# mhnazeri/PMoE

Hardware: AMD Instinct MI355X
Metric: samples/sec fwd+bwd, 256x256 RGB 4-expert PMoE (higher is better)
Workload: dtype bf16; 1 GPU; 4-expert MoE (PMoE experts), 256x256x3 x4 frames, batch 64/GPU, fwd+moe_loss+bwd, dropout 0.3; global_batch=64, parallelism=dp1

## Files before the change

include/pmoe_hip.h:

```cpp
#ifndef PMOE_HIP_H
#define PMOE_HIP_H
#include <stdint.h>
#ifdef __cplusplus
extern "C" {
#endif

#define PMOE_DT_BF16 0
#define PMOE_DT_F32 1

#define PMOE_ERR_ARG (-1)
#define PMOE_ERR_UNSUPPORTED (-2)

#define PMOE_ACT_NONE 0
#define PMOE_ACT_RELU 1
#define PMOE_ACT_ELU 2
#define PMOE_ACT_TANH 3
#define PMOE_ACT_SIGMOID 4

#define PMOE_RES_NONE 0
#define PMOE_RES_ADD 1
#define PMOE_RES_DRELU 2
#define PMOE_RES_DELU 3
#define PMOE_RES_DTANH 4
#define PMOE_RES_DSIGMOID 5
// ... 90 lines not shown
                  float* part, int32_t nparts, float* shiftc, int32_t dtype, void* stream);
int pmoe_reduce_partials(const float* part_in, float* part_out, int32_t E, int32_t nin, int32_t nout, int32_t width,
                         void* stream);
int pmoe_bn_finalize(const float* part, int32_t nparts, int64_t count, const void* const* gamma_ptrs,
                     const void* const* beta_ptrs, void* const* rmean_ptrs, void* const* rvar_ptrs, float momentum,
                     float eps, int32_t training, float* scale, float* shift, float* mean, float* invstd, int32_t E,
                     int32_t C, const float* shiftc, void* stream);
int pmoe_bn_apply(const void* x, const void* res, void* y, const float* scale, const float* shift, const float* mean,
                  int64_t rows_per_expert, int32_t E, int32_t C, int32_t relu, int32_t y_ld, int32_t y_coff,
                  int32_t dtype, void* y_fp8, float in_scale, void* stream);
int pmoe_bn_apply_gap(const void* x, void* y, const float* scale, const float* shift, const float* mean, float* gap_part,
                      int32_t nparts, int32_t N, int32_t ipe, int64_t HW, int32_t C, int32_t relu, int32_t dtype, void* stream);
int pmoe_bn_bwd_reduce(const void* dy, const void* y, const void* x, const float* mean, const float* invstd,
                       const float* scale, const float* shift, int64_t rows_per_expert, int32_t E, int32_t C, int32_t relu, float* part, int32_t nparts,
                       void* gmask_out, int32_t dtype, void* stream);
int pmoe_bn_bwd_finalize(const float* part, int32_t nparts, int64_t count, float* dgamma, float* dbeta, float* c1,
                         float* c2, int32_t E, int32_t C, void* stream);
int pmoe_bn_apply_pool2(const void* x, void* y, void* pooled, const float* scale, const float* shift, const float* mean,
                        int32_t ipe, int32_t H, int32_t W, int32_t E, int32_t C, int32_t relu, int32_t y_ld, int32_t y_coff,
                        int32_t dtype, void* stream);
int pmoe_bn_bwd_apply(const void* dy, const void* y, const void* x, const float* mean, const float* invstd,
                      const float* scale, const float* shift, const float* c1, const float* c2, void* dx, void* gmask_out,
                      int64_t rows_per_expert, int32_t E, int32_t C, int32_t relu, int32_t dtype, void* stream);

int pmoe_maxpool3s2_fwd(const void* x, void* y, uint8_t* argmax, int32_t N, int32_t H, int32_t W, int32_t C,
                        int32_t dtype, void* stream);
int pmoe_maxpool3s2_bwd(const void* dy, const uint8_t* argmax, void* dx, int32_t N, int32_t H, int32_t W, int32_t C,
                        int32_t dtype, void* stream);
int pmoe_gap_partial(const void* a, const void* b, float* part, int32_t N, int64_t HW, int32_t C, int32_t nparts,
                     int32_t b_shared_ipe, int32_t dtype, void* stream);
int pmoe_gap_finish(const float* part, void* out, int32_t N, int32_t C, int32_t nparts, int64_t HW, int32_t out_ld,
                    int32_t out_coff, int32_t dtype, void* stream);
int pmoe_gap_bwd(const void* g, void* dx, int32_t N, int64_t HW, int32_t C, int32_t g_ld, int32_t g_coff,
                 int32_t dtype, void* stream);

int pmoe_stem_tail_stats(const void* z2, const float* sc2, const float* sh2, const float* mu2, float* part,
                         int32_t nparts, float* shiftc, float* part_x, int32_t E, int32_t ipe, int32_t H, int32_t W,
                         int32_t C, int32_t dtype, void* stream);
int pmoe_stem_tail_pool(const void* z2, void* y, uint8_t* argmax, const float* sc2, const float* sh2, const float* sc1,
                        const float* sh1, const float* mu2, const float* mu1, int32_t N, int32_t ipe, int32_t H, int32_t W, int32_t C, int32_t dtype,
                        void* stream);
int pmoe_stem_tail_bwd(int32_t phase, const void* z2, const void* dpool, const uint8_t* argmax, void* dz2,
                       const float* const* consts, float* part, int32_t nparts, int32_t E, int32_t ipe, int32_t H,
                       int32_t W, int32_t C, int32_t dtype, void* stream);
int pmoe_stem_tail_pooled(const void* y, const void* dpool, const uint8_t* argmax, const float* const* consts,
                          float* part4, int32_t nparts, int32_t E, int64_t rows_per_expert, int32_t C, int32_t dtype,
// ... 107 lines not shown
```

pmoe_amd/csrc/elementwise.hip:

```cpp
#include "common.h"

#define DISPATCH_DT(dtype, CALL)                      \
    do {                                              \
        if ((dtype) == PMOE_DT_BF16) { using T = bf16; CALL; } \
        else if ((dtype) == PMOE_DT_F32) { using T = float; CALL; } \
        else return PMOE_ERR_ARG;                     \
    } while (0)

static inline bool pow2(int v) { return v > 0 && !(v & (v - 1)); }

template <typename T, int MODE>
__global__ void __launch_bounds__(256) colstats_kernel(const T* __restrict__ x, const T* __restrict__ dy,
                                                      const T* __restrict__ y, const float* __restrict__ mean,
                                                      const float* __restrict__ invstd, const float* __restrict__ scale,
                                                      const float* __restrict__ shift, long long rpe, int C, int ld,
                                                      int coff, int relu, float* __restrict__ part, int nparts,
                                                      float* __restrict__ shiftc, T* __restrict__ gmask) {
    constexpr int VE = 16 / (int)sizeof(T);
    const int CV = C / VE, RL = 256 / CV;
    const int tid = threadIdx.x, cv = tid % CV, rl = tid / CV;
    const int e = blockIdx.y, pi = blockIdx.x;
    const long long rpp = (rpe + nparts - 1) / nparts;
    long long r0 = (long long)pi * rpp, r1 = r0 + rpp;
    if (r1 > rpe) r1 = rpe;
// ... 249 lines not shown
    }
    const bool remask = relu && !y;
    for (long long i = i0; i < nvec; i += (long long)gridDim.x * 256) {
        const size_t off = ebase + (size_t)i * VE;
        float gv[VE], xv[VE], o[VE];
        unpack16<T>(ldg16(dy + off), gv);
        unpack16<T>(ldg16(x + off), xv);
        if (remask) {
#pragma unroll
            for (int k = 0; k < VE; ++k) gv[k] = ((xv[k] - mu[k]) * sc[k] + sh[k]) > 0.f ? gv[k] : 0.f;
        } else if (relu) {
            float yv[VE];
            unpack16<T>(ldg16(y + off), yv);
#pragma unroll
            for (int k = 0; k < VE; ++k) gv[k] = yv[k] > 0.f ? gv[k] : 0.f;
        }
#pragma unroll
        for (int k = 0; k < VE; ++k) o[k] = gv[k] * A[k] + ((xv[k] - mu[k]) * Bx[k] + K[k]);
        stg16(dx + off, pack16<T>(o));
        if (gm) stg16(gm + off, pack16<T>(gv));
    }
}

template <typename T>
__global__ void __launch_bounds__(256) bn_apply_pool2_kernel(const T* __restrict__ x, T* __restrict__ y, T* __restrict__ pooled,
                                                            const float* __restrict__ scale, const float* __restrict__ shift,
                                                            const float* __restrict__ mean, int ipe, int H, int W, int C, int relu,
                                                            int y_ld, int y_coff) {
    constexpr int VE = 16 / (int)sizeof(T);
    const int CV = C / VE;
    const int e = blockIdx.y, Ho = H / 2, Wo = W / 2;
    const long long nq = (long long)ipe * Ho * Wo * CV;
    const long long i0 = (long long)blockIdx.x * 256 + threadIdx.x;
    const int cv = (int)(i0 % CV);
    float sc[VE], sh[VE], mu[VE];
#pragma unroll
    for (int k = 0; k < VE; ++k) {
        sc[k] = scale[e * C + cv * VE + k]; sh[k] = shift[e * C + cv * VE + k]; mu[k] = mean[e * C + cv * VE + k];
    }
    const size_t rpe = (size_t)ipe * H * W;
    for (long long i = i0; i < nq; i += (long long)gridDim.x * 256) {
        long long t = i / CV;
        const int ox = (int)(t % Wo); t /= Wo;
        const int oy = (int)(t % Ho);
        const int n = (int)(t / Ho);
        const size_t r00 = (size_t)e * rpe + ((size_t)n * H + 2 * oy) * W + 2 * ox;
// ... 485 lines not shown
        const long long nq = (long long)ipe * (H / 2) * (W / 2) * (C / VE);
        hipLaunchKernelGGL((bn_apply_pool2_kernel<T>), dim3(grid_for(nq, 2048), E), dim3(256), 0, (hipStream_t)stream, (const T*)x,
                           (T*)y, (T*)pooled, scale, shift, mean, ipe, H, W, C, relu, y_ld, y_coff);
        return (int)hipGetLastError();
    });
}

int pmoe_bn_bwd_apply(const void* dy, const void* y, const void* x, const float* mean, const float* invstd,
                      const float* scale, const float* shift, const float* c1, const float* c2, void* dx, void* gmask_out,
                      int64_t rows_per_expert, int32_t E, int32_t C, int32_t relu, int32_t dtype, void* stream) {
    DISPATCH_DT(dtype, {
        constexpr int VE = 16 / (int)sizeof(T);
        if (C % VE || !pow2(C / VE) || C / VE > 256) return PMOE_ERR_ARG;
        const long long nvec = rows_per_expert * (C / VE);
        int cap = 1024 / (E > 0 ? E : 1);
        cap = cap < 64 ? 64 : cap;
        hipLaunchKernelGGL((bn_bwd_apply_kernel<T>), dim3(grid_for(nvec, cap), E), dim3(256), 0, (hipStream_t)stream,
                           (const T*)dy, (const T*)y, (const T*)x, mean, invstd, scale, shift, c1, c2, (T*)dx, (T*)gmask_out,
                           (long long)rows_per_expert, C, relu);
        return (int)hipGetLastError();
    });
}

int pmoe_act_fwd(const void* x, void* y, int64_t n, int32_t act, float drop_p, uint64_t seed, int32_t dtype, void* stream) {
    if (!x || !y || n <= 0 || act < PMOE_ACT_NONE || act > PMOE_ACT_SIGMOID || drop_p < 0.f || drop_p >= 1.f) return PMOE_ERR_ARG;
    DISPATCH_DT(dtype, {
        constexpr int VE = 16 / (int)sizeof(T);
        if (n % VE) return PMOE_ERR_ARG;
        hipLaunchKernelGGL((act_fwd_kernel<T>), dim3(grid_for(n / VE)), dim3(256), 0, (hipStream_t)stream, (const T*)x, (T*)y,
                           (long long)(n / VE), act, drop_p, (unsigned long long)seed);
        return (int)hipGetLastError();
    });
}

int pmoe_act_bwd(const void* dy, const void* y, void* dx, int64_t n, int32_t act, float drop_p, int32_t dtype, void* stream) {
    if (!dy || !y || !dx || n <= 0 || act < PMOE_ACT_NONE || act > PMOE_ACT_SIGMOID || drop_p < 0.f || drop_p >= 1.f) return PMOE_ERR_ARG;
    DISPATCH_DT(dtype, {
        constexpr int VE = 16 / (int)sizeof(T);
        if (n % VE) return PMOE_ERR_ARG;
        hipLaunchKernelGGL((act_bwd_kernel<T>), dim3(grid_for(n / VE)), dim3(256), 0, (hipStream_t)stream, (const T*)dy,
                           (const T*)y, (T*)dx, (long long)(n / VE), act, drop_p);
        return (int)hipGetLastError();
    });
}

int pmoe_maxpool3s2_fwd(const void* x, void* y, uint8_t* argmax, int32_t N, int32_t H, int32_t W, int32_t C,
// ... 136 lines not shown
```

pmoe_amd/engine.py:

```python
import itertools
import os

import torch
import torch.distributed as dist

from . import hip, ops
from .model import blocks as B
from .parallel import BucketedAllReduce

F32 = torch.float32


def r16(c):
    return (c + 15) // 16 * 16


def r64(c):
    return (c + 63) // 64 * 64


class Var:
    __slots__ = ("t", "coff", "c", "g", "needs_grad", "act", "drop_p", "base", "gap_part", "bn_src", "bn_part", "f8", "bn_defer",
                 "bn_fused", "pending_bn")

# ... 105 lines not shown
    def __init__(self, experts, alt=False, shared_k=0):
        self.experts = list(experts)
        self.E = len(self.experts)
        self.alt = alt
        self.shared = shared_k > 0
        self.K = shared_k if self.shared else self.E
        if self.shared and (self.E != 1 or alt or 5 * self.K > 64):
            raise ValueError("shared-trunk mixture: one trunk, plain alpha head, n_experts <= 12")
        self.dp_group = None
        self.dp_enabled = False
        self.dp_buckets = 6
        self.dp_always = False
        self._built_for = None
        self._seed_counter = itertools.count(1)
        self.fuse_conv_stats = True
        self.fuse_stem_tail = True
        self.fold_stem_input = True
        self.overlap_wgrad = os.environ.get("PMOE_OVERLAP_WGRAD", "0") == "1"
        self.fold_bn_eval = True
        self.pooled_stem_bwd = True
        self.fold_eca_gate = True
        self.bn_mask_in_reduce = os.environ.get("PMOE_BN_MASK_IN_REDUCE", "1") != "0"
        self.bn_reduce_in_dgrad = os.environ.get("PMOE_BN_REDUCE_IN_DGRAD", "1") != "0"
        self.fuse_bn_gap = os.environ.get("PMOE_FUSE_BN_GAP", "1") != "0"
        self.stem_bn_fuse = os.environ.get("PMOE_STEM_BN_FUSE", "1") != "0"
        self.mlp_wgrad_fused = os.environ.get("PMOE_MLP_WGRAD", "1") != "0"
        self.fp8 = False
        self.fp8_in_scale = 16.0
        self.fp8_min_cin = int(os.environ.get("PMOE_FP8_MIN_CIN", "64"))
        self.raw_alpha = False
        self.debug_grads = None
        self.debug_acts = None
        self._collect()

    def _collect(self):
        ex = self.experts
        self.params = []

        def conv(name, mods, ks=None):
            m0 = mods[0]
            if isinstance(m0, B.Linear):
                layer = GroupedConv(self, name, [m.weight for m in mods],
                                    [m.bias for m in mods] if m0.bias is not None else None,
                                    m0.in_features, m0.out_features, 1, 1, 0)
            else:
                layer = GroupedConv(self, name, [m.weight for m in mods],
# ... 472 lines not shown
        if gm is not None:
            if dz is not None:
                ops.set_meta(name=layer.name, bytes=nb * 3)
                ops.bn_bwd_apply(gm, None, z.t, mean, invstd, scale, shift, c1, c2, dz, None, rpe, E, C_, False)
        else:
            gm = torch.empty_like(z.t) if want_res else None
            if dz is None and gm is None:
                return
            if dz is None:
                dz = torch.empty_like(z.t)
            ops.set_meta(name=layer.name, bytes=nb * (2 + (ysrc is not None) + 1 + (gm is not None)))
            ops.bn_bwd_apply(dy, ysrc, z.t, mean, invstd, scale, shift, c1, c2, dz, gm, rpe, E, C_, relu)
        if self.debug_grads is not None:
            self.debug_grads[layer.name + ":dz"] = dz.detach().clone()
            self.debug_grads[layer.name + ":stats"] = (mean.clone(), invstd.clone(), c1.clone(), c2.clone())
        if z.needs_grad:
            if z.grad is not None:
                raise RuntimeError("BN input consumed twice")
            z.set_grad(dz)
        if want_res:
            if res.grad is not None:
                raise RuntimeError("residual gradient slot already filled")
            res.set_grad(gm)

    def _bn_grad_views(self, layer):
        return (self._grad_slot("gamma", layer).view(self.E, layer.C), self._grad_slot("beta", layer).view(self.E, layer.C),
                None)

    def _stem_tail(self, z2, stats):
        E, C_ = self.E, self.bn_c2.C
        n, h, w, _ = z2.t.shape
        rpe = self.B * h * w
        sc2, sh2, mu2, is2 = self._bn_coeffs(self.bn_c2, rpe, stats, stats.shape[0] // E if stats is not None else 0, z2)
        nparts = self._nparts(rpe)
        part = part_x = None
        if self.training:
            part = torch.empty(E, nparts, 2, C_, dtype=F32, device=self.dev)
            shc = torch.empty(E, C_, dtype=F32, device=self.dev)
            if self.taping:
                part_x = torch.empty(E, nparts, 3, C_, dtype=F32, device=self.dev)
            ops.stem_tail_stats(z2.t, sc2, sh2, mu2, part, nparts, E, self.B, shiftc=shc, part_x=part_x)
            if part_x is not None:
                part_x, npx = self._fold_parts(part_x, nparts, 3 * C_)
        sc1, sh1, mu1, is1 = self._bn_coeffs(self.bn1, rpe, part, nparts, shiftc=shc if self.training else None)
        ho, wo = (h - 1) // 2 + 1, (w - 1) // 2 + 1
        y = Var(self._new(n, ho, wo, C_))
# ... 320 lines not shown
            z1.needs_grad = True
            z1.bn_defer = (self.stem_bn_fuse and self.training and self.bn_reduce_in_dgrad and self.dtype == torch.bfloat16
                           and fold2 and ops.conv2d_wgrad(x0.t, z1.t, None, cin=self.conv1.cinp, cout=self.conv1.cout_st,
                                                          cinp=64, coutp=64, ipe=self.B, ks=3, stride=1, pad=self.conv1.pad,
                                                          x_shared=True, per_image=True, bn_fuse=(z1.t, None, None, None),
                                                          plan_only=True) == 7209)
            self.tape.append(lambda: self._stem_in_bwd(x0, z1, gate, gapmean))
            a1 = self._bn(z1, self.bn_c1, relu=True, stats=st, want_gap=fold2)
        else:
            x0s = self._eca(x0, self.eca1, shared=True)
            a1 = self._conv_bn(x0s, self.conv1, self.bn_c1, relu=True)
        if fold2:
            z2, st = self._eca_conv_folded(a1, self.eca2, self.conv2)
        else:
            a1s = self._eca(a1, self.eca2, shared=False)
            z2, st = self._conv_stats(a1s, self.conv2)
        if self.fuse_stem_tail:
            o = self._stem_tail(z2, st)
        else:
            a2 = self._bn(z2, self.bn_c2, relu=True, stats=st)
            a3 = self._bn(a2, self.bn1, relu=True)
            o = self._maxpool(a3)
        for bi, blk in enumerate(self.blocks):
            idn = o
            if blk["down"] is not None:
                idn = self._conv_bn(o, blk["down"][0], blk["down"][1], relu=False)
            nxt = self.blocks[bi + 1]["conv1"] if bi + 1 < len(self.blocks) else None
            aA = self._conv_bn(o, blk["conv1"], blk["bn1"], relu=True, want_f8=blk["conv2"].fp8)
            o = self._conv_bn(aA, blk["conv2"], blk["bn2"], relu=True, res=idn, want_f8=nxt is not None and nxt.fp8)
        self._gap_to(o, feat, 0)

    def _conv_bn(self, x, conv, bn, relu, res=None, out=None, want_f8=False, pool_to=None):
        if self.training or self.taping or not self.fold_bn_eval or conv.w_f8 is not None:
            z, st = self._conv_stats(x, conv)
            return self._bn(z, bn, relu=relu, res=res, stats=st, out=out, want_f8=want_f8, pool_to=pool_to)
        E = self.E
        key = (self.dtype, str(self.dev)) + tuple(p._version for p in conv.weights) + tuple(
            v for m in bn.mods for v in (m.weight._version, m.bias._version, m.running_mean._version, m.running_var._version))
        cache = conv.__dict__.get("_bn_fold")
        if cache is None or cache[0] != key:
            scale, shift, mean, _ = self._bn_coeffs(bn, 1)
            wf = torch.empty(E, conv.coutp, conv.taps, conv.cinp, dtype=self.dtype, device=self.dev)
            bf = torch.empty(E, conv.coutp, dtype=F32, device=self.dev)
            ops.pack_conv_weights_scaled(self._tab("w", conv), scale, shift, mean, wf, bf, E, conv.cout, conv.cin, conv.ks,
                                         conv.coutp, conv.cinp, self.dtype)
            cache = conv.__dict__["_bn_fold"] = (key, wf, bf)
        _, wf, bf = cache
        H, W = x.t.shape[1], x.t.shape[2]
        Ho = ops.conv_out_size(H, conv.ks, conv.stride, conv.pad)
        Wo = ops.conv_out_size(W, conv.ks, conv.stride, conv.pad)
        o = Var(self._new(self.N, Ho, Wo, conv.cout_st), conv.cout_st, 0) if out is None else out.window(0, conv.cout_st)
        ops.set_meta(flop=2.0 * self.N * Ho * Wo * conv.cout * conv.cin * conv.taps, name=conv.name + "+bn")
# ... 167 lines not shown
```

pmoe_amd/hip.py:

```python
import ctypes as C
import os
from pathlib import Path

import torch

_LIB_PATH = Path(os.environ.get("PMOE_HIP_LIB") or Path(__file__).resolve().parent / "libpmoe_hip.so")
_lib = None

ABI_VERSION = 401
DT_BF16, DT_F32 = 0, 1
ACT_NONE, ACT_RELU, ACT_ELU, ACT_TANH, ACT_SIGMOID = 0, 1, 2, 3, 4
RES_NONE, RES_ADD, RES_DRELU, RES_DELU, RES_DTANH, RES_DSIGMOID, RES_DBN, RES_INBN = 0, 1, 2, 3, 4, 5, 6, 7
ERR_ARG, ERR_UNSUPPORTED = -1, -2
RES_OF_ACT = {ACT_RELU: RES_DRELU, ACT_ELU: RES_DELU, ACT_TANH: RES_DTANH, ACT_SIGMOID: RES_DSIGMOID}
ACT_BY_NAME = {"relu": ACT_RELU, "elu": ACT_ELU, "tanh": ACT_TANH, "sigmoid": ACT_SIGMOID}

_TORCH_DT = {torch.bfloat16: DT_BF16, torch.float32: DT_F32}


class HipUnavailable(RuntimeError):
    pass


class ConvDesc(C.Structure):
# ... 38 lines not shown
    "pmoe_conv2d_stat_rows": [C.POINTER(ConvDesc)],
    "pmoe_conv2d_plan": [C.POINTER(ConvDesc)],
    "pmoe_conv2d_wgrad": [C.POINTER(WgradDesc), _P],
    "pmoe_conv2d_wgrad_fold": [C.POINTER(WgradDesc), _P],
    "pmoe_conv2d_wgrad_ws_floats": [C.POINTER(WgradDesc)],
    "pmoe_conv2d_wgrad_plan": [C.POINTER(WgradDesc)],
    "pmoe_mlp_wgrad": [_P, _P, _P, _P, _I, _I, _I, _I, _I, _I, _I, _I, _I, _I, _I, _I, _P],
    "pmoe_bn_apply_pool2": [_P, _P, _P, _P, _P, _P, _I, _I, _I, _I, _I, _I, _I, _I, _I, _P],
    "pmoe_pack_conv_weights": [_P, _P, _P, _I, _I, _I, _I, _I, _I, _I, _I, _I, _P],
    "pmoe_pack_conv_weights_fp8": [_P, _P, _P, _P, _P, _F, _I, _I, _I, _I, _I, _I, _I, _I, _P],
    "pmoe_pack_conv_weights_scaled": [_P, _P, _P, _P, _P, _P, _I, _I, _I, _I, _I, _I, _I, _P],
    "pmoe_pack_conv_weights_gated": [_P, _P, _I, _P, _P, _I, _I, _I, _I, _I, _I, _I, _I, _I, _I, _P],
    "pmoe_unpack_conv_wgrad": [_P, _P, _I, _I, _I, _I, _I, _I, _P],
    "pmoe_pack_bias": [_P, _P, _I, _I, _I, _P],
    "pmoe_act_fwd": [_P, _P, _L, _I, _F, C.c_uint64, _I, _P],
    "pmoe_act_bwd": [_P, _P, _P, _L, _I, _F, _I, _P],
    "pmoe_colstats": [_P, _L, _I, _I, _I, _I, _P, _I, _P, _I, _P],
    "pmoe_reduce_partials": [_P, _P, _I, _I, _I, _I, _P],
    "pmoe_bn_finalize": [_P, _I, _L, _P, _P, _P, _P, _F, _F, _I, _P, _P, _P, _P, _I, _I, _P, _P],
    "pmoe_bn_apply": [_P, _P, _P, _P, _P, _P, _L, _I, _I, _I, _I, _I, _I, _P, _F, _P],
    "pmoe_bn_bwd_reduce": [_P, _P, _P, _P, _P, _P, _P, _L, _I, _I, _I, _P, _I, _P, _I, _P],
    "pmoe_bn_bwd_finalize": [_P, _I, _L, _P, _P, _P, _P, _I, _I, _P],
    "pmoe_bn_bwd_apply": [_P, _P, _P, _P, _P, _P, _P, _P, _P, _P, _P, _L, _I, _I, _I, _I, _P],
    "pmoe_stem_tail_stats": [_P, _P, _P, _P, _P, _I, _P, _P, _I, _I, _I, _I, _I, _I, _P],
    "pmoe_stem_tail_pooled": [_P, _P, _P, C.POINTER(C.c_void_p), _P, _I, _I, _L, _I, _I, _P],
    "pmoe_stem_tail_combine": [_P, _I, _P, _I, C.POINTER(C.c_void_p), _L, _P, _P, _I, _I, _P],
    "pmoe_stem_tail_pool": [_P, _P, _P, _P, _P, _P, _P, _P, _P, _I, _I, _I, _I, _I, _I, _P],
    "pmoe_stem_tail_bwd": [_I, _P, _P, _P, _P, C.POINTER(C.c_void_p), _P, _I, _I, _I, _I, _I, _I, _I, _P],
    "pmoe_maxpool3s2_fwd": [_P, _P, _P, _I, _I, _I, _I, _I, _P],
    "pmoe_maxpool3s2_bwd": [_P, _P, _P, _I, _I, _I, _I, _I, _P],
    "pmoe_gap_partial": [_P, _P, _P, _I, _L, _I, _I, _I, _I, _P],
    "pmoe_bn_apply_gap": [_P, _P, _P, _P, _P, _P, _I, _I, _I, _L, _I, _I, _I, _P],
    "pmoe_gap_finish": [_P, _P, _I, _I, _I, _L, _I, _I, _I, _P],
    "pmoe_gap_bwd": [_P, _P, _I, _L, _I, _I, _I, _I, _P],
    "pmoe_eca_gate": [_P, _I, _L, _P, _I, _P, _P, _I, _I, _I, _I, _I, _P],
    "pmoe_eca_scale": [_P, _P, _P, _I, _L, _I, _I, _I, _P],
    "pmoe_eca_bwd_small": [_P, _I, _P, _P, _P, _I, _P, _P, _P, _I, _I, _I, _I, _F, _P],
    "pmoe_eca_stem_fold": [_P, _P, _P, _P, _P, _I, _I, _I, _I, _I, _I, _I, _I, _P],
    "pmoe_eca_bwd_apply": [_P, _P, _P, _P, _I, _L, _I, _I, _P],
    "pmoe_nchw_to_nhwc": [_P, _P, _I, _I, _I, _I, _I, _I, _P],
    "pmoe_pad_rows": [_P, _P, _I, _I, _I, _I, _P],
    "pmoe_gate_mixture_fwd": [_P, _I, _P, _I, _P, _P, _P, _P, _I, _I, _I, _I, _I, _P],
    "pmoe_gate_mixture_bwd": [_P, _I, _P, _P, _P, _P, _P, _P, _P, _I, _I, _I, _I, _I, _I, _P],
    "pmoe_moe_loss": [_P, _P, _P, _P, _P, _P, _F, _F, _P, _P, _P, _P, _P, _P, _I, _I, _I, _P],
    "pmoe_maxpool2s2_fwd": [_P, _P, _I, _I, _I, _I, _I, _I, _I, _P],
    "pmoe_pixel_shuffle2": [_P, _P, _I, _I, _I, _I, _I, _I, _I, _I, _P],
# ... 135 lines not shown
```

pmoe_amd/ops.py:

```python
import ctypes as C

import torch

from . import hip
from .hip import ConvDesc, WgradDesc, check, dt, load, ptr, stream_ptr


def _round_up(v, m):
    return (v + m - 1) // m * m


def conv_out_size(h, ks, stride, pad):
    return (h + 2 * pad - ks) // stride + 1


def _nhwc(t, name):
    if t.dim() != 4:
        raise ValueError(f"{name}: expected NHWC [N,H,W,C], got shape {tuple(t.shape)}")
    return t.shape


def _conv_desc(n, h, w_, ho, wo, cin, cout, coutp, ipe, ks, stride, pad, dtype, *, dilate=False, in_shared=False, in_ld=0,
               in_coff=0, out_ld=0, out_coff=0, res_mode=hip.RES_NONE, res_ld=0, res_coff=0, act=hip.ACT_NONE, drop_p=0.0, seed=0,
               w_fp8=False, in_fp8=False, in_scale=1.0, bn_ipe=0, shuffle2_c=0):
# ... 256 lines not shown
        raise ValueError("bn_apply_pool2: x [E*ipe,H,W,C], y [E*ipe,H,W,ld], pooled [E*ipe,H/2,W/2,C]")
    check(load().pmoe_bn_apply_pool2(ptr(x, "x"), ptr(y, "y", x.dtype), ptr(pooled, "pooled", x.dtype), ptr(scale), ptr(shift),
                                     ptr(mean, "mean", torch.float32), ipe, h, w_, E, C_, int(relu), y.shape[-1], y_coff, dt(x),
                                     stream_ptr()), "pmoe_bn_apply_pool2")


def bn_bwd_reduce(dy, y, x, mean, invstd, scale, shift, rpe, E, C_, relu, part, nparts, gmask=None):
    check(load().pmoe_bn_bwd_reduce(ptr(dy, "dy"), ptr(y, "y", dy.dtype), ptr(x, "x", dy.dtype), ptr(mean), ptr(invstd),
                                    ptr(scale), ptr(shift), rpe, E, C_, int(relu), ptr(part, "part", torch.float32), nparts,
                                    ptr(gmask, "gmask", dy.dtype), dt(dy), stream_ptr()), "pmoe_bn_bwd_reduce")


def bn_bwd_finalize(part, nparts, count, dgamma, dbeta, c1, c2, E, C_):
    check(load().pmoe_bn_bwd_finalize(ptr(part), nparts, count, ptr(dgamma), ptr(dbeta), ptr(c1), ptr(c2), E, C_,
                                      stream_ptr()), "pmoe_bn_bwd_finalize")


def bn_bwd_apply(dy, y, x, mean, invstd, scale, shift, c1, c2, dx, gmask, rpe, E, C_, relu):
    check(load().pmoe_bn_bwd_apply(ptr(dy, "dy"), ptr(y, "y", dy.dtype), ptr(x, "x", dy.dtype), ptr(mean), ptr(invstd),
                                   ptr(scale), ptr(shift), ptr(c1), ptr(c2), ptr(dx, "dx", dy.dtype), ptr(gmask, "gmask", dy.dtype),
                                   rpe, E, C_, int(relu), dt(dy), stream_ptr()), "pmoe_bn_bwd_apply")


def stem_tail_stats(z2, sc2, sh2, mu2, part, nparts, E, ipe, shiftc=None, part_x=None):
    n, h, w_, c = _nhwc(z2, "z2")
    check(load().pmoe_stem_tail_stats(ptr(z2, "z2"), ptr(sc2), ptr(sh2), ptr(mu2), ptr(part, "part", torch.float32), nparts,
                                      ptr(shiftc, "shiftc", torch.float32), ptr(part_x, "part_x", torch.float32), E, ipe,
                                      h, w_, c, dt(z2), stream_ptr()), "pmoe_stem_tail_stats")


def _consts12(consts):
    return (C.c_void_p * 12)(*[t.data_ptr() if t is not None else None for t in consts])


def stem_tail_pooled(y, dpool, argmax, consts, part4, nparts, E):
    n, ho, wo, c = _nhwc(y, "y")
    check(load().pmoe_stem_tail_pooled(ptr(y, "y"), ptr(dpool, "dpool", y.dtype), ptr(argmax, "argmax", torch.uint8),
                                       _consts12(consts), ptr(part4, "part4", torch.float32), nparts, E,
                                       (n // E) * ho * wo, c, dt(y), stream_ptr()), "pmoe_stem_tail_pooled")


def stem_tail_combine(part4, np4, part_x, npx, consts, count, out1, out2, E, c):
    f32 = torch.float32
    check(load().pmoe_stem_tail_combine(ptr(part4, "part4", f32), np4, ptr(part_x, "part_x", f32), npx, _consts12(consts),
                                        count, ptr(out1, "out1", f32), ptr(out2, "out2", f32), E, c, stream_ptr()),
          "pmoe_stem_tail_combine")
# ... 148 lines not shown


def _timed(fn):
    @_functools.wraps(fn)
    def wrapper(*a, **k):
        global _next_meta
        if _prof is None:
            return fn(*a, **k)
        meta, _next_meta = _next_meta, {}
        e0, e1 = torch.cuda.Event(enable_timing=True), torch.cuda.Event(enable_timing=True)
        e0.record()
        r = fn(*a, **k)
        e1.record()
        if _launch_info:
            meta.update(_launch_info)
            _launch_info.clear()
        _prof.append((fn.__name__, meta, e0, e1))
        return r
    return wrapper


for _n in ("stem_tail_stats", "stem_tail_pool", "stem_tail_bwd", "stem_tail_pooled", "stem_tail_combine", "conv2d", "conv2d_wgrad", "conv2d_wgrad_fold", "pack_conv_weights", "pack_conv_weights_scaled", "pack_conv_weights_gated", "unpack_conv_wgrad", "pack_bias", "colstats",
           "reduce_partials", "bn_finalize", "bn_apply", "bn_apply_gap", "bn_bwd_reduce", "bn_bwd_finalize", "bn_bwd_apply",
           "maxpool_fwd", "maxpool_bwd", "gap_partial", "gap_finish", "gap_bwd", "eca_gate", "eca_scale",
           "eca_bwd_small", "eca_bwd_apply", "eca_stem_fold", "nchw_to_nhwc", "pad_rows", "gate_mixture_fwd", "gate_mixture_bwd",
           "moe_loss"):
    globals()[_n] = _timed(globals()[_n])


def maxpool2_fwd(x, y, c=None, x_coff=0):
    n, h, w_, ld = _nhwc(x, "x")
    c = ld if c is None else c
    if tuple(y.shape) != (n, h // 2, w_ // 2, c):
        raise ValueError(f"maxpool2_fwd: y must be {(n, h // 2, w_ // 2, c)}, got {tuple(y.shape)}")
    check(load().pmoe_maxpool2s2_fwd(ptr(x, "x"), ptr(y, "y", x.dtype), n, h, w_, c, ld, x_coff, dt(x), stream_ptr()),
          "pmoe_maxpool2s2_fwd")


def pixel_shuffle2(src, dst, c, dst_coff=0):
    n, h, w_, sld = _nhwc(src, "src")
    n2, h2, w2, dld = _nhwc(dst, "dst")
    if (n2, h2, w2) != (n, 2 * h, 2 * w_):
        raise ValueError(f"pixel_shuffle2: dst must be [{n},{2 * h},{2 * w_},*], got {tuple(dst.shape)}")
    check(load().pmoe_pixel_shuffle2(ptr(src, "src"), ptr(dst, "dst", src.dtype), n, h, w_, c, sld, dld, dst_coff, dt(src),
                                     stream_ptr()), "pmoe_pixel_shuffle2")

# ... 141 lines not shown
```

Measured before the change: 1923 samples/s.

## Fuse downsample BN into residual BN-add-ReLU with packed ReLU mask bits

Adds kernels that apply the conv2 BN, the downsample-branch BN, the residual add and the ReLU in one pass, and write a one-byte-per-vector ReLU mask instead of relying on re-reading y. The backward reduce masks dy using these bits and collects BN gradient statistics for both branches at once. A paired apply kernel then writes both input gradients in a single pass. The aim is to avoid materialising the normalised downsample output and to cut separate elementwise launches and memory traffic in residual blocks. In exchange it adds more code paths and extra partial buffers for the fold and finalize steps.

Result: faster. 1962 samples/s, median of 6 (+2.0%).

```diff
diff --git a/include/pmoe_hip.h b/include/pmoe_hip.h
--- a/include/pmoe_hip.h
+++ b/include/pmoe_hip.h
@@ -136,6 +136,14 @@
 int pmoe_bn_bwd_apply(const void* dy, const void* y, const void* x, const float* mean, const float* invstd,
                       const float* scale, const float* shift, const float* c1, const float* c2, void* dx, void* gmask_out,
                       int64_t rows_per_expert, int32_t E, int32_t C, int32_t relu, int32_t dtype, void* stream);
+int pmoe_bn_res_apply(const void* x, const float* coef, const void* res, const void* res_z, const float* res_coef, void* y,
+                      uint8_t* relu_bits, int64_t rows_per_expert, int32_t E, int32_t C, int32_t dtype, void* stream);
+int pmoe_bn_bwd_reduce_res(const void* dy, const void* y, const uint8_t* relu_bits, const void* x, const float* coef,
+                           const void* ds_z, const float* ds_coef, float* part, float* ds_part, int32_t nparts, void* g_out,
+                           int64_t rows_per_expert, int32_t E, int32_t C, int32_t dtype, void* stream);
+int pmoe_bn_bwd_apply_pair(const void* g, const void* x, const float* coef, const float* c1, const float* c2, void* dx,
+                           const void* ds_z, const float* ds_coef, const float* ds_c1, const float* ds_c2, void* ds_dz,
+                           int64_t rows_per_expert, int32_t E, int32_t C, int32_t dtype, void* stream);
 
 int pmoe_maxpool3s2_fwd(const void* x, void* y, uint8_t* argmax, int32_t N, int32_t H, int32_t W, int32_t C,
                         int32_t dtype, void* stream);
diff --git a/pmoe_amd/csrc/elementwise.hip b/pmoe_amd/csrc/elementwise.hip
--- a/pmoe_amd/csrc/elementwise.hip
+++ b/pmoe_amd/csrc/elementwise.hip
@@ -295,6 +295,161 @@
     }
 }
 
+template <typename T, bool DS>
+__global__ void __launch_bounds__(256) bn_res_apply_kernel(const T* __restrict__ x, const float* __restrict__ coef,
+                                                          const T* __restrict__ res, const float* __restrict__ rcoef,
+                                                          T* __restrict__ y, unsigned char* __restrict__ bits, long long rpe, int C) {
+    constexpr int VE = 16 / (int)sizeof(T);
+    const int CV = C / VE;
+    const int e = blockIdx.y, EC = (int)gridDim.y * C;
+    const long long nvec = rpe * CV;
+    const size_t ebase = (size_t)e * rpe * C;
+    const long long i0 = (long long)blockIdx.x * 256 + threadIdx.x;
+    const int cv = (int)(i0 % CV);
+    float sc[VE], sh[VE], mu[VE], rsc[VE], rsh[VE], rmu[VE];
+#pragma unroll
+    for (int k = 0; k < VE; ++k) {
+        const int c = e * C + cv * VE + k;
+        mu[k] = coef[c]; sc[k] = coef[2 * EC + c]; sh[k] = coef[3 * EC + c];
+        rmu[k] = DS ? rcoef[c] : 0.f; rsc[k] = DS ? rcoef[2 * EC + c] : 0.f; rsh[k] = DS ? rcoef[3 * EC + c] : 0.f;
+    }
+    for (long long i = i0; i < nvec; i += (long long)gridDim.x * 256) {
+        float xv[VE], rv[VE];
+        const size_t off = ebase + (size_t)i * VE;
+        unpack16<T>(ldg16(x + off), xv);
+        unpack16<T>(ldg16(res + off), rv);
+        if (DS) {
+#pragma unroll
+            for (int k = 0; k < VE; ++k) rv[k] = (rv[k] - rmu[k]) * rsc[k] + rsh[k];
+            unpack16<T>(pack16<T>(rv), rv);
+        }
+#pragma unroll
+        for (int k = 0; k < VE; ++k) xv[k] = (xv[k] - mu[k]) * sc[k] + sh[k];
+#pragma unroll
+        for (int k = 0; k < VE; ++k) xv[k] += rv[k];
+#pragma unroll
+        for (int k = 0; k < VE; ++k) xv[k] = fmaxf(xv[k], 0.f);
+        const v4i pk = pack16<T>(xv);
+        stg16(y + off, pk);
+        if (bits) {
+            float yv[VE];
+            unpack16<T>(pk, yv);
+            unsigned m = 0;
+#pragma unroll
+            for (int k = 0; k < VE; ++k) m |= (yv[k] > 0.f ? 1u : 0u) << k;
+            bits[(size_t)e * nvec + i] = (unsigned char)m;
+        }
+    }
+}
+
+template <typename T, bool DS>
+__global__ void __launch_bounds__(256) bn_bwd_reduce_res_kernel(const T* __restrict__ dy, const T* __restrict__ y,
+                                                               const unsigned char* __restrict__ bits, const T* __restrict__ x,
+                                                               const float* __restrict__ coef, const T* __restrict__ xd,
+                                                               const float* __restrict__ dcoef, long long rpe, int C,
+                                                               float* __restrict__ part, float* __restrict__ dpart, int nparts,
+                                                               T* __restrict__ gout) {
+    constexpr int VE = 16 / (int)sizeof(T);
+    const int CV = C / VE, RL = 256 / CV;
+    const int tid = threadIdx.x, cv = tid % CV, rl = tid / CV;
+    const int e = blockIdx.y, pi = blockIdx.x, EC = (int)gridDim.y * C;
+    const long long rpp = (rpe + nparts - 1) / nparts;
+    long long r0 = (long long)pi * rpp, r1 = r0 + rpp;
+    if (r1 > rpe) r1 = rpe;
+    float s1[VE], s2[VE], s3[VE], mu[VE], is[VE], dmu[VE], dis[VE];
+#pragma unroll
+    for (int i = 0; i < VE; ++i) {
+        const int c = e * C + cv * VE + i;
+        s1[i] = s2[i] = s3[i] = 0.f;
+        mu[i] = coef[c]; is[i] = coef[EC + c];
+        dmu[i] = DS ? dcoef[c] : 0.f; dis[i] = DS ? dcoef[EC + c] : 0.f;
+    }
+    const size_t ebase = (size_t)e * rpe;
+    for (long long r = r0 + rl; r < r1; r += RL) {
+        const size_t off = (ebase + r) * C + cv * VE;
+        float xv[VE], gv[VE];
+        unpack16<T>(ldg16(x + off), xv);
+        unpack16<T>(ldg16(dy + off), gv);
+        if (bits) {
+            const unsigned m = bits[(ebase + r) * CV + cv];
+#pragma unroll
+            for (int i = 0; i < VE; ++i) gv[i] = ((m >> i) & 1u) ? gv[i] : 0.f;
+        } else {
+            float yv[VE];
+            unpack16<T>(ldg16(y + off), yv);
+#pragma unroll
+            for (int i = 0; i < VE; ++i) gv[i] = yv[i] > 0.f ? gv[i] : 0.f;
+        }
+        stg16(gout + off, pack16<T>(gv));
+#pragma unroll
+        for (int i = 0; i < VE; ++i) { s1[i] += gv[i]; s2[i] += gv[i] * (xv[i] - mu[i]) * is[i]; }
+        if (DS) {
+            float dv[VE];
+            unpack16<T>(ldg16(xd + off), dv);
+#pragma unroll
+            for (int i = 0; i < VE; ++i) s3[i] += gv[i] * (dv[i] - dmu[i]) * dis[i];
+        }
+    }
+    __shared__ float red[DS ? 3 : 2][256 * 8];
+#pragma unroll
+    for (int i = 0; i < VE; ++i) {
+        red[0][rl * C + cv * VE + i] = s1[i];
+        red[1][rl * C + cv * VE + i] = s2[i];
+        if (DS) red[DS ? 2 : 0][rl * C + cv * VE + i] = s3[i];
+    }
+    __syncthreads();
+    for (int c = tid; c < (DS ? 3 : 2) * C; c += 256) {
+        const int which = c / C, cc = c % C;
+        float s = 0.f;
+        for (int k = 0; k < RL; ++k) s += red[which][k * C + cc];
+        const size_t row = ((size_t)e * nparts + pi) * 2;
+        if (which < 2) part[(row + which) * C + cc] = s;
+        if (DS && which != 1) dpart[(row + (which >> 1)) * C + cc] = s;
+    }
+}
+
+template <typename T>
+__global__ void __launch_bounds__(256) bn_bwd_apply_pair_kernel(const T* __restrict__ g, const T* __restrict__ x,
+                                                               const float* __restrict__ coef, const float* __restrict__ c1,
+                                                               const float* __restrict__ c2, T* __restrict__ dx,
+                                                               const T* __restrict__ xd, const float* __restrict__ dcoef,
+                                                               const float* __restrict__ dc1, const float* __restrict__ dc2,
+                                                               T* __restrict__ dxd, long long rpe, int C) {
+    constexpr int VE = 16 / (int)sizeof(T);
+    const int CV = C / VE;
+    const int e = blockIdx.y, EC = (int)gridDim.y * C;
+    const long long nvec = rpe * CV;
+    const size_t ebase = (size_t)e * rpe * C;
+    const long long i0 = (long long)blockIdx.x * 256 + threadIdx.x;
+    const int cv = (int)(threadIdx.x & (CV - 1));
+    float A[VE], Bx[VE], K[VE], mu[VE], dA[VE], dBx[VE], dK[VE], dmu[VE];
+#pragma unroll
+    for (int k = 0; k < VE; ++k) {
+        const int c = e * C + cv * VE + k;
+        mu[k] = coef[c];
+        A[k] = coef[2 * EC + c];
+        Bx[k] = -A[k] * coef[EC + c] * c2[c];
+        K[k] = -A[k] * c1[c];
+        dmu[k] = dcoef[c];
+        dA[k] = dcoef[2 * EC + c];
+        dBx[k] = -dA[k] * dcoef[EC + c] * dc2[c];
+        dK[k] = -dA[k] * dc1[c];
+    }
+    for (long long i = i0; i < nvec; i += (long long)gridDim.x * 256) {
+        const size_t off = ebase + (size_t)i * VE;
+        float gv[VE], xv[VE], dv[VE], o[VE];
+        unpack16<T>(ldg16(g + off), gv);
+        unpack16<T>(ldg16(x + off), xv);
+        unpack16<T>(ldg16(xd + off), dv);
+#pragma unroll
+        for (int k = 0; k < VE; ++k) o[k] = gv[k] * A[k] + ((xv[k] - mu[k]) * Bx[k] + K[k]);
+        stg16(dx + off, pack16<T>(o));
+#pragma unroll
+        for (int k = 0; k < VE; ++k) o[k] = gv[k] * dA[k] + ((dv[k] - dmu[k]) * dBx[k] + dK[k]);
+        stg16(dxd + off, pack16<T>(o));
+    }
+}
+
 template <typename T>
 __global__ void __launch_bounds__(256) bn_apply_pool2_kernel(const T* __restrict__ x, T* __restrict__ y, T* __restrict__ pooled,
                                                             const float* __restrict__ scale, const float* __restrict__ shift,
@@ -826,6 +981,63 @@
     });
 }
 
+int pmoe_bn_res_apply(const void* x, const float* coef, const void* res, const void* res_z, const float* res_coef, void* y,
+                      uint8_t* relu_bits, int64_t rows_per_expert, int32_t E, int32_t C, int32_t dtype, void* stream) {
+    if (!x || !coef || !y || rows_per_expert < 1 || E < 1 || (res != nullptr) == (res_z != nullptr) || (res_z && !res_coef))
+        return PMOE_ERR_ARG;
+    DISPATCH_DT(dtype, {
+        constexpr int VE = 16 / (int)sizeof(T);
+        if (C % VE || !pow2(C / VE) || C / VE > 256) return PMOE_ERR_ARG;
+        const dim3 grid(grid_for(rows_per_expert * (C / VE), 2048), E);
+        if (res_z)
+            hipLaunchKernelGGL((bn_res_apply_kernel<T, true>), grid, dim3(256), 0, (hipStream_t)stream, (const T*)x, coef,
+                               (const T*)res_z, res_coef, (T*)y, relu_bits, (long long)rows_per_expert, C);
+        else
+            hipLaunchKernelGGL((bn_res_apply_kernel<T, false>), grid, dim3(256), 0, (hipStream_t)stream, (const T*)x, coef,
+                               (const T*)res, nullptr, (T*)y, relu_bits, (long long)rows_per_expert, C);
+        return (int)hipGetLastError();
+    });
+}
+
+int pmoe_bn_bwd_reduce_res(const void* dy, const void* y, const uint8_t* relu_bits, const void* x, const float* coef,
+                           const void* ds_z, const float* ds_coef, float* part, float* ds_part, int32_t nparts, void* g_out,
+                           int64_t rows_per_expert, int32_t E, int32_t C, int32_t dtype, void* stream) {
+    if (!dy || !x || !coef || !part || !g_out || nparts < 1 || rows_per_expert < 1 || E < 1 || (y != nullptr) == (relu_bits != nullptr) ||
+        (ds_z && (!ds_coef || !ds_part)))
+        return PMOE_ERR_ARG;
+    DISPATCH_DT(dtype, {
+        constexpr int VE = 16 / (int)sizeof(T);
+        if (C % VE || !pow2(C / VE) || C / VE > 256) return PMOE_ERR_ARG;
+        const dim3 grid(nparts, E);
+        if (ds_z)
+            hipLaunchKernelGGL((bn_bwd_reduce_res_kernel<T, true>), grid, dim3(256), 0, (hipStream_t)stream, (const T*)dy, (const T*)y,
+                               relu_bits, (const T*)x, coef, (const T*)ds_z, ds_coef, (long long)rows_per_expert, C, part, ds_part,
+                               nparts, (T*)g_out);
+        else
+            hipLaunchKernelGGL((bn_bwd_reduce_res_kernel<T, false>), grid, dim3(256), 0, (hipStream_t)stream, (const T*)dy, (const T*)y,
+                               relu_bits, (const T*)x, coef, nullptr, nullptr, (long long)rows_per_expert, C, part, nullptr, nparts,
+                               (T*)g_out);
+        return (int)hipGetLastError();
+    });
+}
+
+int pmoe_bn_bwd_apply_pair(const void* g, const void* x, const float* coef, const float* c1, const float* c2, void* dx,
+                           const void* ds_z, const float* ds_coef, const float* ds_c1, const float* ds_c2, void* ds_dz,
+                           int64_t rows_per_expert, int32_t E, int32_t C, int32_t dtype, void* stream) {
+    if (!g || !x || !coef || !c1 || !c2 || !dx || !ds_z || !ds_coef || !ds_c1 || !ds_c2 || !ds_dz || rows_per_expert < 1 || E < 1)
+        return PMOE_ERR_ARG;
+    DISPATCH_DT(dtype, {
+        constexpr int VE = 16 / (int)sizeof(T);
+        if (C % VE || !pow2(C / VE) || C / VE > 256) return PMOE_ERR_ARG;
+        int cap = 1024 / E;
+        cap = cap < 64 ? 64 : cap;
+        hipLaunchKernelGGL((bn_bwd_apply_pair_kernel<T>), dim3(grid_for(rows_per_expert * (C / VE), cap), E), dim3(256), 0,
+                           (hipStream_t)stream, (const T*)g, (const T*)x, coef, c1, c2, (T*)dx, (const T*)ds_z, ds_coef, ds_c1,
+                           ds_c2, (T*)ds_dz, (long long)rows_per_expert, C);
+        return (int)hipGetLastError();
+    });
+}
+
 int pmoe_act_fwd(const void* x, void* y, int64_t n, int32_t act, float drop_p, uint64_t seed, int32_t dtype, void* stream) {
     if (!x || !y || n <= 0 || act < PMOE_ACT_NONE || act > PMOE_ACT_SIGMOID || drop_p < 0.f || drop_p >= 1.f) return PMOE_ERR_ARG;
     DISPATCH_DT(dtype, {
diff --git a/pmoe_amd/engine.py b/pmoe_amd/engine.py
--- a/pmoe_amd/engine.py
+++ b/pmoe_amd/engine.py
@@ -151,6 +151,8 @@
         self.fold_eca_gate = True
         self.bn_mask_in_reduce = os.environ.get("PMOE_BN_MASK_IN_REDUCE", "1") != "0"
         self.bn_reduce_in_dgrad = os.environ.get("PMOE_BN_REDUCE_IN_DGRAD", "1") != "0"
+        self.bn_ds_fuse = os.environ.get("PMOE_BN_DS_FUSE", "1") != "0"
+        self.bn_maskbits = os.environ.get("PMOE_BN_MASKBITS", "1") != "0"
         self.fuse_bn_gap = os.environ.get("PMOE_FUSE_BN_GAP", "1") != "0"
         self.stem_bn_fuse = os.environ.get("PMOE_STEM_BN_FUSE", "1") != "0"
         self.mlp_wgrad_fused = os.environ.get("PMOE_MLP_WGRAD", "1") != "0"
@@ -669,6 +671,83 @@
             if res.grad is not None:
                 raise RuntimeError("residual gradient slot already filled")
             res.set_grad(gm)
+
+    def _res_tail_ok(self):
+        return ((self.training or self.taping) and not self.fp8 and self.debug_acts is None and self.debug_grads is None
+                and self.bn_mask_in_reduce)
+
+    def _bn_res(self, z, layer, stats, res, ds):
+        E, C_ = self.E, layer.C
+        n, h, w, _ = z.t.shape
+        rpe = self.B * h * w
+        if stats is not None and stats.shape[2] != C_:
+            raise RuntimeError("fused stats width mismatch")
+        self._bn_coeffs(layer, rpe, stats, stats.shape[0] // E if stats is not None else 0, z)
+        coef = self._last_coef
+        y = Var(torch.empty_like(z.t))
+        y.needs_grad = (z.needs_grad or layer.trainable or
+                        ((ds[0].needs_grad or ds[1].trainable) if ds is not None else res.needs_grad))
+        taped = self.taping and y.needs_grad
+        bits = ops.relu_bits_like(y.t) if taped and self.bn_maskbits else None
+        ops.set_meta(name=layer.name, bytes=z.t.numel() * z.t.element_size() * 3 + (bits.numel() if bits is not None else 0))
+        if ds is not None:
+            ops.bn_res_apply(z.t, coef, None, ds[0].t, ds[2], y.t, bits, rpe, E, C_)
+        else:
+            ops.bn_res_apply(z.t, coef, res.t, None, None, y.t, bits, rpe, E, C_)
+        if taped:
+            train = self.training
+            self.tape.append(lambda: self._bn_res_bwd(z, layer, y, res, ds, coef, bits, rpe, train))
+        return y
+
+    def _bn_bwd_coeffs(self, layer, part, nparts, rpe, train):
+        E, C_ = self.E, layer.C
+        part, nparts = self._fold_parts(part, nparts, 2 * C_, cap=2048)
+        c1, c2 = (torch.empty(E, C_, dtype=F32, device=self.dev) for _ in range(2))
+        dgamma, dbeta, store = self._bn_grad_views(layer)
+        ops.bn_bwd_finalize(part, nparts, rpe, dgamma, dbeta, c1, c2, E, C_)
+        if store is not None:
+            store()
+        if not train:
+            c1.zero_()
+            c2.zero_()
+        return c1, c2
+
+    def _bn_res_bwd(self, z, layer, y, res, ds, coef, bits, rpe, train):
+        dy = y.grad
+        if dy is None:
+            return
+        E, C_ = self.E, layer.C
+        nb = z.t.numel() * z.t.element_size()
+        zd, dlayer, dcoef = ds if ds is not None else (None, None, None)
+        nparts = self._nparts(rpe)
+        part = torch.empty(E, nparts, 2, C_, dtype=F32, device=self.dev)
+        dpart = torch.empty_like(part) if ds is not None else None
+        g = torch.empty_like(z.t)
+        ops.set_meta(name=layer.name, bytes=nb * (3 + (ds is not None)) + (bits.numel() if bits is not None else nb))
+        ops.bn_bwd_reduce_res(dy, y.t if bits is None else None, bits, z.t, coef, zd.t if ds is not None else None, dcoef,
+                              part, dpart, nparts, g, rpe, E, C_)
+        c1, c2 = self._bn_bwd_coeffs(layer, part, nparts, rpe, train)
+        if z.needs_grad and z.grad is not None or (ds is not None and zd.needs_grad and zd.grad is not None):
+            raise RuntimeError("BN input consumed twice")
+        if ds is not None:
+            dc1, dc2 = self._bn_bwd_coeffs(dlayer, dpart, nparts, rpe, train)
+            if z.needs_grad and zd.needs_grad:
+                dz, dzd = torch.empty_like(z.t), torch.empty_like(zd.t)
+                ops.set_meta(name=layer.name, bytes=nb * 5)
+                ops.bn_bwd_apply_pair(g, z.t, coef, c1, c2, dz, zd.t, dcoef, dc1, dc2, dzd, rpe, E, C_)
+                z.set_grad(dz)
+                zd.set_grad(dzd)
+                return
+        for v, cf, k1, k2 in ((z, coef, c1, c2),) + (((zd, dcoef, dc1, dc2),) if ds is not None else ()):
+            if v.needs_grad:
+                dv = torch.empty_like(v.t)
+                ops.set_meta(name=layer.name, bytes=nb * 3)
+                ops.bn_bwd_apply(g, None, v.t, cf[0], cf[1], cf[2], cf[3], k1, k2, dv, None, rpe, E, C_, False)
+                v.set_grad(dv)
+        if ds is None and res.needs_grad:
+            if res.grad is not None:
+                raise RuntimeError("residual gradient slot already filled")
+            res.set_grad(g)
 
     def _bn_grad_views(self, layer):
         return (self._grad_slot("gamma", layer).view(self.E, layer.C), self._grad_slot("beta", layer).view(self.E, layer.C),
@@ -1035,12 +1114,23 @@
             a3 = self._bn(a2, self.bn1, relu=True)
             o = self._maxpool(a3)
         for bi, blk in enumerate(self.blocks):
-            idn = o
+            idn, ds = o, None
+            tail = self._res_tail_ok()
             if blk["down"] is not None:
-                idn = self._conv_bn(o, blk["down"][0], blk["down"][1], relu=False)
+                if tail and self.bn_ds_fuse:
+                    zd, std = self._conv_stats(o, blk["down"][0])
+                    self._bn_coeffs(blk["down"][1], self.B * zd.t.shape[1] * zd.t.shape[2], std,
+                                    std.shape[0] // self.E if std is not None else 0, zd)
+                    idn, ds = None, (zd, blk["down"][1], self._last_coef)
+                else:
+                    idn = self._conv_bn(o, blk["down"][0], blk["down"][1], relu=False)
             nxt = self.blocks[bi + 1]["conv1"] if bi + 1 < len(self.blocks) else None
             aA = self._conv_bn(o, blk["conv1"], blk["bn1"], relu=True, want_f8=blk["conv2"].fp8)
-            o = self._conv_bn(aA, blk["conv2"], blk["bn2"], relu=True, res=idn, want_f8=nxt is not None and nxt.fp8)
+            if ds is not None or (tail and self.bn_maskbits and self.taping and idn.needs_grad):
+                z2, st2 = self._conv_stats(aA, blk["conv2"])
+                o = self._bn_res(z2, blk["bn2"], st2, idn, ds)
+            else:
+                o = self._conv_bn(aA, blk["conv2"], blk["bn2"], relu=True, res=idn, want_f8=nxt is not None and nxt.fp8)
         self._gap_to(o, feat, 0)
 
     def _conv_bn(self, x, conv, bn, relu, res=None, out=None, want_f8=False, pool_to=None):
diff --git a/pmoe_amd/hip.py b/pmoe_amd/hip.py
--- a/pmoe_amd/hip.py
+++ b/pmoe_amd/hip.py
@@ -84,6 +84,9 @@
     "pmoe_bn_bwd_reduce": [_P, _P, _P, _P, _P, _P, _P, _L, _I, _I, _I, _P, _I, _P, _I, _P],
     "pmoe_bn_bwd_finalize": [_P, _I, _L, _P, _P, _P, _P, _I, _I, _P],
     "pmoe_bn_bwd_apply": [_P, _P, _P, _P, _P, _P, _P, _P, _P, _P, _P, _L, _I, _I, _I, _I, _P],
+    "pmoe_bn_res_apply": [_P, _P, _P, _P, _P, _P, _P, _L, _I, _I, _I, _P],
+    "pmoe_bn_bwd_reduce_res": [_P, _P, _P, _P, _P, _P, _P, _P, _P, _I, _P, _L, _I, _I, _I, _P],
+    "pmoe_bn_bwd_apply_pair": [_P, _P, _P, _P, _P, _P, _P, _P, _P, _P, _P, _L, _I, _I, _I, _P],
     "pmoe_stem_tail_stats": [_P, _P, _P, _P, _P, _I, _P, _P, _I, _I, _I, _I, _I, _I, _P],
     "pmoe_stem_tail_pooled": [_P, _P, _P, C.POINTER(C.c_void_p), _P, _I, _I, _L, _I, _I, _P],
     "pmoe_stem_tail_combine": [_P, _I, _P, _I, C.POINTER(C.c_void_p), _L, _P, _P, _I, _I, _P],
diff --git a/pmoe_amd/ops.py b/pmoe_amd/ops.py
--- a/pmoe_amd/ops.py
+++ b/pmoe_amd/ops.py
@@ -302,6 +302,57 @@
                                    rpe, E, C_, int(relu), dt(dy), stream_ptr()), "pmoe_bn_bwd_apply")
 
 
+def _coef_block(coef, E, C_, name):
+    if coef is not None and (coef.dtype != torch.float32 or tuple(coef.shape) != (4, E, C_)):
+        raise ValueError(f"{name}: expected the f32 block [mean | invstd | scale | shift] of shape {(4, E, C_)}")
+    return ptr(coef, name, torch.float32)
+
+
+def relu_bits_like(y):
+    return torch.empty(y.numel() * y.element_size() // 16, dtype=torch.uint8, device=y.device)
+
+
+def bn_res_apply(x, coef, res, res_z, res_coef, y, relu_bits, rpe, E, C_):
+    if tuple(x.shape) != tuple(y.shape) or x.numel() != E * rpe * C_:
+        raise ValueError("bn_res_apply: x, y dense [E*rpe, C]")
+    for t, n in ((res, "res"), (res_z, "res_z")):
+        if t is not None and tuple(t.shape) != tuple(x.shape):
+            raise ValueError(f"bn_res_apply: {n} must have x's shape")
+    if relu_bits is not None and relu_bits.numel() * 16 != y.numel() * y.element_size():
+        raise ValueError("bn_res_apply: relu_bits holds one byte per 16 bytes of y")
+    check(load().pmoe_bn_res_apply(ptr(x, "x"), _coef_block(coef, E, C_, "coef"), ptr(res, "res", x.dtype),
+                                   ptr(res_z, "res_z", x.dtype), _coef_block(res_coef, E, C_, "res_coef"), ptr(y, "y", x.dtype),
+                                   ptr(relu_bits, "relu_bits", torch.uint8), rpe, E, C_, dt(x), stream_ptr()), "pmoe_bn_res_apply")
+
+
+def bn_bwd_reduce_res(dy, y, relu_bits, x, coef, ds_z, ds_coef, part, ds_part, nparts, g_out, rpe, E, C_):
+    if dy.numel() != E * rpe * C_ or any(t is not None and tuple(t.shape) != tuple(dy.shape) for t in (y, x, ds_z, g_out)):
+        raise ValueError("bn_bwd_reduce_res: dy, y, x, ds_z, g_out dense [E*rpe, C]")
+    if relu_bits is not None and relu_bits.numel() * 16 != dy.numel() * dy.element_size():
+        raise ValueError("bn_bwd_reduce_res: relu_bits holds one byte per 16 bytes of y")
+    for p, n in ((part, "part"), (ds_part, "ds_part")):
+        if p is not None and p.numel() != E * nparts * 2 * C_:
+            raise ValueError(f"bn_bwd_reduce_res: {n} must be [E, nparts, 2, C]")
+    check(load().pmoe_bn_bwd_reduce_res(ptr(dy, "dy"), ptr(y, "y", dy.dtype), ptr(relu_bits, "relu_bits", torch.uint8),
+                                        ptr(x, "x", dy.dtype), _coef_block(coef, E, C_, "coef"), ptr(ds_z, "ds_z", dy.dtype),
+                                        _coef_block(ds_coef, E, C_, "ds_coef"), ptr(part, "part", torch.float32),
+                                        ptr(ds_part, "ds_part", torch.float32), nparts, ptr(g_out, "g_out", dy.dtype), rpe, E, C_,
+                                        dt(dy), stream_ptr()), "pmoe_bn_bwd_reduce_res")
+
+
+def bn_bwd_apply_pair(g, x, coef, c1, c2, dx, ds_z, ds_coef, ds_c1, ds_c2, ds_dz, rpe, E, C_):
+    if g.numel() != E * rpe * C_ or any(tuple(t.shape) != tuple(g.shape) for t in (x, dx, ds_z, ds_dz)):
+        raise ValueError("bn_bwd_apply_pair: g, x, dx, ds_z, ds_dz dense [E*rpe, C]")
+    f32 = torch.float32
+    for t in (c1, c2, ds_c1, ds_c2):
+        if t.numel() != E * C_:
+            raise ValueError("bn_bwd_apply_pair: c1 / c2 are [E, C]")
+    check(load().pmoe_bn_bwd_apply_pair(ptr(g, "g"), ptr(x, "x", g.dtype), _coef_block(coef, E, C_, "coef"), ptr(c1, "c1", f32),
+                                        ptr(c2, "c2", f32), ptr(dx, "dx", g.dtype), ptr(ds_z, "ds_z", g.dtype),
+                                        _coef_block(ds_coef, E, C_, "ds_coef"), ptr(ds_c1, "ds_c1", f32), ptr(ds_c2, "ds_c2", f32),
+                                        ptr(ds_dz, "ds_dz", g.dtype), rpe, E, C_, dt(g), stream_ptr()), "pmoe_bn_bwd_apply_pair")
+
+
 def stem_tail_stats(z2, sc2, sh2, mu2, part, nparts, E, ipe, shiftc=None, part_x=None):
     n, h, w_, c = _nhwc(z2, "z2")
     check(load().pmoe_stem_tail_stats(ptr(z2, "z2"), ptr(sc2), ptr(sh2), ptr(mu2), ptr(part, "part", torch.float32), nparts,
@@ -496,6 +547,7 @@
 
 for _n in ("stem_tail_stats", "stem_tail_pool", "stem_tail_bwd", "stem_tail_pooled", "stem_tail_combine", "conv2d", "conv2d_wgrad", "conv2d_wgrad_fold", "pack_conv_weights", "pack_conv_weights_scaled", "pack_conv_weights_gated", "unpack_conv_wgrad", "pack_bias", "colstats",
            "reduce_partials", "bn_finalize", "bn_apply", "bn_apply_gap", "bn_bwd_reduce", "bn_bwd_finalize", "bn_bwd_apply",
+           "bn_res_apply", "bn_bwd_reduce_res", "bn_bwd_apply_pair",
            "maxpool_fwd", "maxpool_bwd", "gap_partial", "gap_finish", "gap_bwd", "eca_gate", "eca_scale",
            "eca_bwd_small", "eca_bwd_apply", "eca_stem_fold", "nchw_to_nhwc", "pad_rows", "gate_mixture_fwd", "gate_mixture_bwd",
            "moe_loss"):
```
